# CompVis/retrieval-augmented-diffusion-models

Hardware: AMD Instinct MI355X
Metric: images/sec at 256x256, 50 DDIM steps, k=4 OpenImages retrieval (higher is better)
Workload: dtype bf16; 1 GPU; BASELINE config #3: RDM sampling, exact kNN (k=4) over a synthetic 20927907 x 512 fp16 CLIP DB -> 50-step DDIM (eta 0, CFG scale 2.0) over the shipped-config UNet (400.9M params, random weights) -> VQ-f4 decode to 256x256; batch_per_gpu=64, global_batch=64, sampler_steps=50, k=4, db_rows=20927907, parallelism=dp1 (batch-sharded, weights + DB replicated, all-gather of images only), deterministic_mode=False

## Files before the change

retrieval-augmented-diffusion-models_amd/csrc/conv_halo4.hip:

```cpp

#include <type_traits>

#include "kernels.h"

__device__ unsigned long long g_halo4_prof[4];

__global__ __launch_bounds__(256) void conv_w_fragpack_kernel(const bf16_t* __restrict__ W, bf16_t* __restrict__ dst, int N, int Cin) {
    const int KQ = Cin >> 4;
    const long long nvec = (long long)N * 9 * Cin / 8;
    for (long long v = (long long)blockIdx.x * 256 + threadIdx.x; v < nvec; v += (long long)gridDim.x * 256) {
        const int lane = (int)(v & 63);
        long long f = v >> 6;
        const int kq = (int)(f % KQ); f /= KQ;
        const int tap = (int)(f % 9); const int nb = (int)(f / 9);
        const int n = nb * 32 + (lane & 31), c = kq * 16 + (lane >> 5) * 8;
        *(uint4*)(dst + v * 8) = *(const uint4*)(W + ((long long)n * 9 + tap) * Cin + c);
    }
}
hipError_t launch_conv_w_fragpack(const bf16_t* W, bf16_t* dst, int N, int Cin, hipStream_t st) {
    const long long nvec = (long long)N * 9 * Cin / 8;
    long long g = (nvec + 255) / 256; if (g > 8192) g = 8192;
    conv_w_fragpack_kernel<<<dim3((unsigned)g), 256, 0, st>>>(W, dst, N, Cin);
    return hipGetLastError();
}
// ... 186 lines not shown
    }
    slice_setup();
    typedef __attribute__((ext_vector_type(4))) unsigned u32x4_t;
    union FragU { u32x4_t u; bf16x8 f; };
    auto start_values = [&](int tm0, int tn0, int row, float (&pb)[FM][FN]) {
#pragma unroll
        for (int i = 0; i < FM; i++) {
            const int mf = tm0 + wm * 128 + i * 32;
            const float* rv = p.rowvec ? p.rowvec + (long long)(mf / p.rows_per_sample) * p.rowvec_ld : nullptr;
#pragma unroll
            for (int j = 0; j < FN; j++) {
                const int ncol = tn0 + wn * WN + j * 32 + row;
                float bv = (S == 1 && p.bias) ? p.bias[ncol] : 0.f;
                if (S == 1 && rv) bv += rv[ncol];
                pb[i][j] = bv;
            }
        }
    };
    auto start_frag = [&](float bv, int half) -> bf16x8 {
        const uint32_t hi = cvt_pk_bf16(bv, 0.f) & 0xffffu;
        const uint32_t lo = cvt_pk_bf16(bv - __uint_as_float(hi << 16), 0.f) & 0xffffu;
        FragU t; t.u = (u32x4_t){half ? 0u : (hi | (lo << 16)), 0u, 0u, 0u};
        return t.f;
    };
    {
        float pb[FM][FN];
        start_values(em0, en0, frow, pb);
        FragU o; o.u = (u32x4_t){fhalf ? 0u : 0x3f803f80u, 0u, 0u, 0u};
        bf16x8 ones = o.f;
#pragma unroll
        for (int i = 0; i < FM; i++) {
            bf16x8 sf[FN];
#pragma unroll
            for (int j = 0; j < FN; j++) sf[j] = start_frag(pb[i][j], fhalf);
            if constexpr (FN == 3) asm volatile("s_nop 7" : "+v"(sf[0]), "+v"(sf[1]), "+v"(sf[2]), "+v"(ones));
            else asm volatile("s_nop 7" : "+v"(sf[0]), "+v"(sf[1]), "+v"(ones));
#pragma unroll
            for (int j = 0; j < FN; j++) H4_MFMA0(i * FN + j, sf[j], ones);
        }
    }

    unsigned long long tprof[2] = {0, 0};
    unsigned long long tp0 = 0, tp1 = 0;
    if (p.dbg & 16) tp0 = __builtin_readcyclecounter();
    bool slice_last_tap = false;
    int epi_stores = 0;
    const char* sbn = Wf; unsigned noff = 0; int q0 = 0;
    auto describe = [&]() {
        slice_last_tap = tap == 8;
        const int n_tap = slice_last_tap ? 0 : tap + 1;
        sbn = slice_last_tap ? sb_after : sb_run + tap_stride;
        sb_run = sbn;
        const int ndy = (n_tap * 11) >> 5, ndx = n_tap - ndy * 3;
        noff = (slice_last_tap ? hbase_nxt : hbase_cur) + (unsigned)(ndy * RSTR + ndx * 144);
        q0 = tap * 3;
    };
    auto step = [&](auto ptag) {
        constexpr int P = decltype(ptag)::value;
        auto mfma = [&](int ks, int m) {
            const int j = m / FM, i = m % FM;
            H4_MFMA(i * FN + j, fb[P][ks][j], fa[ks & 1][i]);
        };
        if (epi_stores == 0) asm volatile("s_waitcnt vmcnt(3) lgkmcnt(0)" ::: "memory");
        else if (epi_stores == FM * ((32 * (WN / 8)) / 64)) asm volatile("s_waitcnt vmcnt(%0) lgkmcnt(0)" :: "i"(3 + FM * ((32 * (WN / 8)) / 64)) : "memory");
        else asm volatile("s_waitcnt vmcnt(%0) lgkmcnt(0)" :: "i"(3 + 4 * FM * FN) : "memory");
        epi_stores = 0;
        H4_LDSW(hdst[P][0], hreg[P][0]);
#pragma unroll
        for (int m = 0; m < FM * FN; m++) {
            mfma(0, m);
            H4_GLOADB(fb[P ^ 1][m / FN][m % FN], voffj[m % FN], sbn, (m / FN) * 1024);
            if (m == 3) {
#pragma unroll
                for (int i = 0; i < FM; i++) H4_LDSR(fa[1][i], va[i], 32);
            }
        }
#pragma unroll
        for (int ks = 1; ks < 4; ks++) {
            asm volatile("s_waitcnt lgkmcnt(0)" ::: "memory");
            if (ks < 3) H4_LDSW(hdst[P][ks], hreg[P][ks]);
            const int q = q0 + ks - 1;
            const bool live = q < hnp;
            unsigned pe;
            asm volatile("ds_read_b32 %0, %1" : "=v"(pe) : "v"(tbl + (unsigned)((q < 20 ? q : 20) * 256)));
            mfma(ks, 0); mfma(ks, 1); mfma(ks, 2); mfma(ks, 3);
            if (ks < 3) {
#pragma unroll
                for (int i = 0; i < FM; i++) H4_LDSR(fa[(ks + 1) & 1][i], va[i], (ks + 1) * 32);
            } else {
                if (slice_last_tap) __builtin_amdgcn_s_barrier();
#pragma unroll
                for (int i = 0; i < FM; i++) { va[i] = vbase[i] + noff; H4_LDSR(fa[0][i], va[i], 0); }
            }
            asm volatile("s_waitcnt lgkmcnt(4)" : "+v"(pe) :: "memory");
            mfma(ks, 4);
            int hy = (int)((pe >> 20) & 63u), sp = (int)((pe >> 26) & 3u), xs = (int)((pe >> 13) & (STRIP ? 127u : 63u));
            if constexpr (STRIP) xs += ht_x0(ht) - 1;
            H4_PIN3(hy, sp, xs);
            mfma(ks, 5);
            int y = ht_y0(ht) + hy - 1;
            const bool xin = STRIP ? ((unsigned)xs < (unsigned)WI) : (((pe >> 19) & 1u) != 0);
            unsigned okm = (live & xin & ((unsigned)y < (unsigned)H)) ? 0xffffffffu : 0u;
            if constexpr (STRIP) xs >>= ups;
            H4_PIN2(y, okm);
            mfma(ks, 6);
            int t = __mul24(ht.b0 + sp, p.Hin) + (y >> ups);
            H4_PIN1(t);
            mfma(ks, 7);
            unsigned pix = (unsigned)__mul24(t, p.Win) + (unsigned)xs;
            unsigned long long ga = (unsigned long long)hs.src + (unsigned long long)pix * hs.ldb + (unsigned)(lc * 16);
            unsigned glo = (unsigned)ga, ghi = (unsigned)(ga >> 32);
            H4_PIN2(glo, ghi);
            if constexpr (FN >= 3) mfma(ks, 8);
            const unsigned long long zb = (unsigned long long)zl;
            glo = (glo & okm) | ((unsigned)zb & ~okm); ghi = (ghi & okm) | ((unsigned)(zb >> 32) & ~okm);
            H4_PIN2(glo, ghi);
            if constexpr (FN >= 3) mfma(ks, 9);
            unsigned hd = hbase_nxt + ((pe & 0x1fffu) << 4);
            hd = (live & (((pe >> 28) & 1u) != 0)) ? hd : dump;
            H4_PIN1(hd);
            const char* hg = (const char*)(((unsigned long long)ghi << 32) | glo);
            if constexpr (FN >= 3) mfma(ks, 10);
            H4_GLOADH(hreg[P][ks - 1], hg); hdst[P][ks - 1] = hd;
            if constexpr (FN >= 3) mfma(ks, 11);
        }
    };
    auto advance = [&]() -> bool {
        if (!slice_last_tap) { tap++; return false; }
        tap = 0; hb ^= 1; sl++;
        if (sl < s_end) { slice_setup(); return false; }

        if (!has_next) asm volatile("s_waitcnt vmcnt(0) lgkmcnt(0)" ::: "memory");
        asm volatile("s_nop 15\n\ts_nop 15" ::: "memory");

        if (p.dbg & 16) { tp1 = __builtin_readcyclecounter(); tprof[0] += tp1 - tp0; }
        char* const stg_base = smem + (hb ^ 1) * HBYTES;
        int lane_e = lane;
        asm volatile("" : "+v"(lane_e));
        const int erow = lane_e & 31, ehalf = lane_e >> 5;
        constexpr int CPR = WN / 8, NIT = (32 * CPR) / 64;
        static_assert((32 * CPR) % 64 == 0, "epilogue staging geometry");
        const bool swz = HBYTES < 4 * 32 * (WN * 4 + 16);
        const int SROW = swz ? WN * 4 : WN * 4 + 16;
        const unsigned stg0 = (unsigned)((hb ^ 1) * HBYTES + wave * 32 * SROW);
        const unsigned fw = swz ? (unsigned)((erow >> 1) & 7) : 0u;
        unsigned stgw[4];
#pragma unroll
        for (int g = 0; g < 4; g++) stgw[g] = stg0 + (unsigned)(erow * SROW) + ((((unsigned)(2 * g + ehalf)) ^ fw) << 4);
        const int eno = en0 + wn * WN;
        float pb[FM][FN];
        start_values(nem0, nen0, erow, pb);
        FragU o1; o1.u = (u32x4_t){ehalf ? 0u : 0x3f803f80u, 0u, 0u, 0u};
        bf16x8 ones = o1.f;
        auto stage_row = [&](int i) {
#pragma unroll
            for (int j = 0; j < FN; j++) {
                H4_LDSW_ACC(stgw[0], i * FN + j, 0, j * 128); H4_LDSW_ACC(stgw[1], i * FN + j, 1, j * 128);
                H4_LDSW_ACC(stgw[2], i * FN + j, 2, j * 128); H4_LDSW_ACC(stgw[3], i * FN + j, 3, j * 128);
            }
            bf16x8 sf[FN];
#pragma unroll
            for (int j = 0; j < FN; j++) sf[j] = start_frag(pb[i][j], ehalf);
            if constexpr (FN == 3) asm volatile("s_waitcnt lgkmcnt(0)\n\ts_nop 7" : "+v"(sf[0]), "+v"(sf[1]), "+v"(sf[2]), "+v"(ones) :: "memory");
            else asm volatile("s_waitcnt lgkmcnt(0)\n\ts_nop 7" : "+v"(sf[0]), "+v"(sf[1]), "+v"(ones) :: "memory");
#pragma unroll
            for (int j = 0; j < FN; j++) H4_MFMA0(i * FN + j, sf[j], ones);
        };
        if (S > 1) {
            constexpr int CPR4 = WN / 4, NIT4 = (32 * CPR4) / 64;
            unsigned voffs[NIT4], lrd4[NIT4];
#pragma unroll
            for (int it = 0; it < NIT4; it++) {
                const int idx = it * 64 + lane_e, row = idx / CPR4, c4 = idx - row * CPR4;
                voffs[it] = (unsigned)(row * p.N + c4 * 4) * 4u;
                const unsigned fr = swz ? (unsigned)((row >> 1) & 7) : 0u;
                lrd4[it] = stg0 + (unsigned)(row * SROW) + ((((unsigned)c4 & ~7u) | (((unsigned)c4 ^ fr) & 7u)) << 4);
            }
            const char* const wbase = (const char*)(p.ws + (long long)part * p.M * p.N + (long long)(em0 + wm * 128) * p.N + eno);
            const unsigned long long rowstep = (unsigned long long)(32 * p.N) * 4ull;
#pragma unroll
            for (int i = 0; i < FM; i++) {
                stage_row(i);
                const char* const op = (const char*)h4_uni64((unsigned long long)(wbase + i * rowstep));
#pragma unroll
                for (int it = 0; it < NIT4; it++) {
                    const float4 a0 = *(const float4*)(smem + lrd4[it]);
                    const h4_u32x4 d0 = {__float_as_uint(a0.x), __float_as_uint(a0.y), __float_as_uint(a0.z), __float_as_uint(a0.w)};
                    H4_GSTORES(voffs[it], d0, op);
                }
            }
        } else {
            unsigned voffs[NIT], lrd[NIT];
#pragma unroll
            for (int it = 0; it < NIT; it++) {
                const int idx = it * 64 + lane_e, row = idx / CPR, ch = idx - row * CPR;
                voffs[it] = (unsigned)(row * p.ldo + ch * 8) * 2u;
                const unsigned fr = swz ? (unsigned)((row >> 1) & 7) : 0u, c4 = (unsigned)(2 * ch);
                lrd[it] = stg0 + (unsigned)(row * SROW) + (((c4 & ~7u) | ((c4 ^ fr) & 7u)) << 4);
            }
            const unsigned lx = swz ? 16u : 0u, la = swz ? 0u : 16u;
            auto frag_row0 = [&](int i) -> long long {
                if constexpr (STRIP) {
                    const int tp = wm * 128 + i * 32;
                    return ((long long)(ht_tile.b0 * H + ht_y0(ht_tile) + (tp >> 6)) * WI + ht_x0(ht_tile) + (tp & 63));
                } else return (long long)(em0 + wm * 128 + i * 32);
            };
            const char* const obase = (const char*)(ob + eno);
            const char* const rbase = (const char*)(rb + eno);
            const unsigned long long rowbytes = (unsigned long long)p.ldo * 2ull;
            h4_u32x4 rr4[2][NIT];
            auto res_request = [&](int i, h4_u32x4 (&dst)[NIT]) {
                const char* const rp = (const char*)h4_uni64((unsigned long long)(rbase + (unsigned long long)frag_row0(i) * rowbytes));
#pragma unroll
                for (int it = 0; it < NIT; it++) H4_GLOADB(dst[it], voffs[it], rp, 0);
            };
            auto res_wait = [&](h4_u32x4 (&r)[NIT], auto ntag) {
                constexpr int N = decltype(ntag)::value;
#pragma unroll
                for (int it = 0; it < NIT; it++) asm volatile("" : "+v"(r[it]));
                asm volatile("s_waitcnt vmcnt(%0)" :: "i"(N) : "memory");
#pragma unroll
                for (int it = 0; it < NIT; it++) asm volatile("" : "+v"(r[it]));
            };
            auto store_row = [&](int i) {
                const char* const op = (const char*)h4_uni64((unsigned long long)(obase + (unsigned long long)frag_row0(i) * rowbytes));
#pragma unroll
                for (int it = 0; it < NIT; it++) {
                    float4 a0 = *(const float4*)(smem + lrd[it]), a1 = *(const float4*)(smem + ((lrd[it] ^ lx) + la));
                    if (rb) {
                        const h4_u32x4 r4 = rr4[i & 1][it];
                        a0.x += __uint_as_float(r4.x << 16); a0.y += __uint_as_float(r4.x & 0xffff0000u);
                        a0.z += __uint_as_float(r4.y << 16); a0.w += __uint_as_float(r4.y & 0xffff0000u);
                        a1.x += __uint_as_float(r4.z << 16); a1.y += __uint_as_float(r4.z & 0xffff0000u);
                        a1.z += __uint_as_float(r4.w << 16); a1.w += __uint_as_float(r4.w & 0xffff0000u);
                    }
                    const h4_u32x4 dv = {cvt_pk_bf16(a0.x, a0.y), cvt_pk_bf16(a0.z, a0.w), cvt_pk_bf16(a1.x, a1.y), cvt_pk_bf16(a1.z, a1.w)};
                    H4_GSTORES(voffs[it], dv, op);
                }
            };
            if (rb) {
                res_request(0, rr4[0]); res_request(1, rr4[1]);
                stage_row(0); res_wait(rr4[0], std::integral_constant<int, NIT>{}); store_row(0);
                res_request(2, rr4[0]);
                stage_row(1); res_wait(rr4[1], std::integral_constant<int, 2 * NIT>{}); store_row(1);
                res_request(3, rr4[1]);
                stage_row(2); res_wait(rr4[0], std::integral_constant<int, 2 * NIT>{}); store_row(2);
                stage_row(3); res_wait(rr4[1], std::integral_constant<int, NIT>{}); store_row(3);
            } else {
                stage_row(0); store_row(0);
                stage_row(1); store_row(1);
                stage_row(2); store_row(2);
                stage_row(3); store_row(3);
            }
        }
        epi_stores = (S > 1) ? 2 * FM * ((32 * (WN / 8)) / 64) : FM * ((32 * (WN / 8)) / 64);
        if (p.dbg & 16) tprof[1] += __builtin_readcyclecounter() - tp1;
        if (!has_next) return true;
        __builtin_amdgcn_s_barrier();
        tile = next;
        tile_setup();
        sl = s_begin;
        slice_setup();
        if (p.dbg & 16) tp0 = __builtin_readcyclecounter();
        return false;
    };
    while (true) {
        describe(); step(std::integral_constant<int, 0>{}); if (advance()) break;
        describe(); step(std::integral_constant<int, 1>{}); if (advance()) break;
    }
    if ((p.dbg & 16) && tid == 0) {
        atomicAdd(&g_halo4_prof[0], tprof[0]); atomicAdd(&g_halo4_prof[1], tprof[1]); atomicAdd(&g_halo4_prof[3], 1ull);
    }
}

template <int FN, bool STRIP = false>
static hipError_t launch_halo4_cfg(const IgemmParams& p, hipStream_t st) {
    constexpr int smem = 2 * H4_HALO_MAX + 4096 + 4 * 21 * 256;
    constexpr int BN = FN * 64;
    static int ncu_dev[RDM_MAX_DEVICES] = {0};
    const int dev = rdm_cur_device();
    if (!ncu_dev[dev]) {
        hipError_t e = hipFuncSetAttribute((const void*)conv3x3_halo4_kernel<FN, STRIP>, hipFuncAttributeMaxDynamicSharedMemorySize, smem);
        if (e != hipSuccess) return e;
        hipDeviceGetAttribute(&ncu_dev[dev], hipDeviceAttributeMultiprocessorCount, dev);
    }
    const int ncu = ncu_dev[dev];
    const long long ntiles = (long long)(p.M / 256) * (p.N / BN) * (p.ksplit > 1 ? p.ksplit : 1);
    long long g = (ncu + 7) & ~7;
    if (g > ntiles) g = ntiles;
    conv3x3_halo4_kernel<FN, STRIP><<<dim3((unsigned)g), 256, smem, st>>>(p);
    return hipGetLastError();
}

hipError_t launch_conv_halo4(const IgemmParams& p, bool strip, hipStream_t st) {
    if (strip) return launch_halo4_cfg<2, true>(p, st);
    if (p.N % 192 == 0) return launch_halo4_cfg<3>(p, st);
    return launch_halo4_cfg<2>(p, st);
}
```

retrieval-augmented-diffusion-models_amd/csrc/h4_asm.h:

```cpp
#pragma once
#include "common.h"

#define H4_ACC0 64
#define H4_ACC_CLOBBERS "a64","a65","a66","a67","a68","a69","a70","a71","a72","a73","a74","a75","a76","a77","a78","a79","a80","a81","a82","a83","a84","a85","a86","a87","a88","a89","a90","a91","a92","a93","a94","a95","a96","a97","a98","a99","a100","a101","a102","a103","a104","a105","a106","a107","a108","a109","a110","a111","a112","a113","a114","a115","a116","a117","a118","a119","a120","a121","a122","a123","a124","a125","a126","a127","a128","a129","a130","a131","a132","a133","a134","a135","a136","a137","a138","a139","a140","a141","a142","a143","a144","a145","a146","a147","a148","a149","a150","a151","a152","a153","a154","a155","a156","a157","a158","a159","a160","a161","a162","a163","a164","a165","a166","a167","a168","a169","a170","a171","a172","a173","a174","a175","a176","a177","a178","a179","a180","a181","a182","a183","a184","a185","a186","a187","a188","a189","a190","a191","a192","a193","a194","a195","a196","a197","a198","a199","a200","a201","a202","a203","a204","a205","a206","a207","a208","a209","a210","a211","a212","a213","a214","a215","a216","a217","a218","a219","a220","a221","a222","a223","a224","a225","a226","a227","a228","a229","a230","a231","a232","a233","a234","a235","a236","a237","a238","a239","a240","a241","a242","a243","a244","a245","a246","a247","a248","a249","a250","a251","a252","a253","a254","a255"
#define H4_MFMA(IDX, a, b)  asm volatile("v_mfma_f32_32x32x16_bf16 a[%c2:%c3], %0, %1, a[%c2:%c3]" :: "v"(a), "v"(b), "i"(H4_ACC0 + (IDX) * 16), "i"(H4_ACC0 + (IDX) * 16 + 15))
#define H4_MFMA0(IDX, a, b) asm volatile("v_mfma_f32_32x32x16_bf16 a[%c2:%c3], %0, %1, 0" :: "v"(a), "v"(b), "i"(H4_ACC0 + (IDX) * 16), "i"(H4_ACC0 + (IDX) * 16 + 15))
#define H4_ACCZERO(IDX, R) asm volatile("v_accvgpr_write_b32 a%c0, 0" :: "i"(H4_ACC0 + (IDX) * 16 + (R)))
#define H4_ACCREAD(dst, IDX, R) asm volatile("v_accvgpr_read_b32 %0, a%c1" : "=v"(dst) : "i"(H4_ACC0 + (IDX) * 16 + (R)))
#define H4_LDSR(dst, addr, off)  asm volatile("ds_read_b128 %0, %1 offset:%2" : "=v"(dst) : "v"(addr), "i"(off))
#define H4_LDSW(addr, src)  asm volatile("ds_write_b128 %0, %1" :: "v"(addr), "v"(src) : "memory")
#define H4_GLOADB(dst, voff, sbase, imm) asm volatile("global_load_dwordx4 %0, %1, %2 offset:%3" : "=v"(dst) : "v"(voff), "s"(sbase), "i"(imm) : "memory")
#define H4_GLOADH(dst, vaddr) asm volatile("global_load_dwordx4 %0, %1, off" : "=v"(dst) : "v"(vaddr) : "memory")
typedef __attribute__((ext_vector_type(4))) unsigned h4_u32x4;
#define H4_GSTORE(vaddr, data) asm volatile("global_store_dwordx4 %0, %1, off\n\ts_nop 1" :: "v"(vaddr), "v"(data) : "memory")
#define H4_PIN1(a) asm volatile("" : "+v"(a))
#define H4_PIN2(a, b) asm volatile("" : "+v"(a), "+v"(b))
#define H4_PIN3(a, b, c) asm volatile("" : "+v"(a), "+v"(b), "+v"(c))
#define H4_GSTOREO(vaddr, data, off) asm volatile("global_store_dwordx4 %0, %1, off offset:%2\n\ts_nop 1" :: "v"(vaddr), "v"(data), "i"(off) : "memory")
#define H4_GSTORES(voff, data, sbase) asm volatile("global_store_dwordx4 %0, %1, %2\n\ts_nop 1" :: "v"(voff), "v"(data), "s"(sbase) : "memory")
#define H4_GSTORES_NT(voff, data, sbase) asm volatile("global_store_dwordx4 %0, %1, %2 nt\n\ts_nop 1" :: "v"(voff), "v"(data), "s"(sbase) : "memory")
#define H4_GSTORESO(voff, data, sbase, off) asm volatile("global_store_dwordx4 %0, %1, %2 offset:%3\n\ts_nop 1" :: "v"(voff), "v"(data), "s"(sbase), "i"(off) : "memory")
__device__ __forceinline__ unsigned long long h4_uni64(unsigned long long v) {
    const unsigned lo = __builtin_amdgcn_readfirstlane((unsigned)v), hi = __builtin_amdgcn_readfirstlane((unsigned)(v >> 32));
    return ((unsigned long long)hi << 32) | lo;
}
#define H4_GLOADB_A(AIDX, voff, sbase) asm volatile("global_load_dwordx4 a[%c0:%c1], %2, %3" :: "i"(AIDX), "i"((AIDX) + 3), "v"(voff), "s"(sbase) : "memory")
#define H4_AREAD(dst, AIDX) asm volatile("v_accvgpr_read_b32 %0, a%c1" : "=v"(dst) : "i"(AIDX))
#define H4_LDSW_ACC(addr, IDX, G, off) asm volatile("ds_write_b128 %0, a[%c1:%c2] offset:%3" :: "v"(addr), "i"(H4_ACC0 + (IDX) * 16 + (G) * 4), "i"(H4_ACC0 + (IDX) * 16 + (G) * 4 + 3), "i"(off) : "memory")
#define H4_ACCWRITE(IDX, R, src) asm volatile("v_accvgpr_write_b32 a%c0, %1" :: "i"(H4_ACC0 + (IDX) * 16 + (R)), "v"(src))
#define H4_LDSWO(addr, src, off)  asm volatile("ds_write_b128 %0, %1 offset:%2" :: "v"(addr), "v"(src), "i"(off) : "memory")
#define H4_PERMSWAP(a, b) asm volatile("v_permlane32_swap_b32 %0, %1" : "+v"(a), "+v"(b))
```

retrieval-augmented-diffusion-models_amd/csrc/lin4.hip:

```cpp

#include <type_traits>

#include "kernels.h"
#include "h4_asm.h"

__host__ __device__ inline int l4_geglu_row(int n) {
    const int nb = n >> 5, fr = n & 31;
    return 64 * (nb >> 1) + 16 * (nb & 1) + (fr < 16 ? fr : 32 + (fr - 16));
}
__global__ __launch_bounds__(256) void lin_w_fragpack_kernel(const bf16_t* __restrict__ W, bf16_t* __restrict__ dst, int N, int K, int ldw, int geglu,
                                                             const float* __restrict__ gamma) {
    const int KQ = K >> 4;
    const long long nvec = (long long)N * K / 8;
    for (long long v = (long long)blockIdx.x * 256 + threadIdx.x; v < nvec; v += (long long)gridDim.x * 256) {
        const int lane = (int)(v & 63);
        const long long f = v >> 6;
        const int kq = (int)(f % KQ), nb = (int)(f / KQ);
        int n = nb * 32 + (lane & 31);
        const int c = kq * 16 + (lane >> 5) * 8;
        if (geglu) n = l4_geglu_row(n);
        uint4 w = *(const uint4*)(W + (long long)n * ldw + c);
        if (gamma) {
            uint32_t* u = (uint32_t*)&w;
#pragma unroll
// ... 153 lines not shown
                const int g = i >= p.N ? 1 : 0, n = i - g * p.N;
                const float bv = ((long long)g * p.rows_per_sample < p.M) ? p.rowvec[(long long)g * p.rowvec_ld + (GEGLU ? l4_geglu_row(n) : n)] : 0.f;
                const uint32_t hi = cvt_pk_bf16(bv, 0.f) & 0xffffu;
                const uint32_t lo = cvt_pk_bf16(bv - __uint_as_float(hi << 16), 0.f) & 0xffffu;
                *(uint32_t*)(smem + L4_RV + i * 4) = hi | (lo << 16);
            }
        }
    }
    __syncthreads();
    typedef __attribute__((ext_vector_type(4))) unsigned u32x4_t;
    union FragU { u32x4_t u; bf16x8 f; };
    auto bias_frags = [&](int bn, int bm, int row, int half, bf16x8 (&bf)[FN], bf16x8& ones) __attribute__((always_inline)) {
        const int rvoff = L4_RV + ((bm * BM >= rv_split) ? p.N * 4 : 0);
#pragma unroll
        for (int j = 0; j < FN; j++) {
            uint32_t w = 0u, w2 = 0u;
            if constexpr (!LN) {
                w = *(const uint32_t*)(smem + L4_BIAS + (bn * BN + wn * WN + j * 32 + row) * 4);
                if (has_rv) w2 = *(const uint32_t*)(smem + rvoff + (bn * BN + wn * WN + j * 32 + row) * 4);
            }
            FragU t; t.u = (u32x4_t){half ? 0u : w, half ? 0u : w2, 0u, 0u};
            bf[j] = t.f;
        }
        FragU o; o.u = (u32x4_t){half ? 0u : 0x3f803f80u, half ? 0u : 0x3f803f80u, 0u, 0u};
        ones = o.f;
    };
    auto acc_init = [&](int bn, int bm) __attribute__((always_inline)) {
        bf16x8 bf[FN], ones;
        bias_frags(bn, bm, frow, fhalf, bf, ones);
        asm volatile("s_nop 7" : "+v"(bf[0]), "+v"(bf[1]), "+v"(bf[2]), "+v"(ones));
#pragma unroll
        for (int i = 0; i < FM; i++)
#pragma unroll
            for (int j = 0; j < FN; j++) H4_MFMA0(i * FN + j, bf[j], ones);
    };

    {
        ASrc s0 = a_src(ca); cur_adv(ca);
#pragma unroll
        for (int q = 0; q < NPC; q++) H4_GLOADB(hreg[0][q], s0.voff, s0.base + (unsigned)q * s0.pstride, 0);
        asm volatile("s_waitcnt vmcnt(0)" ::: "memory");
#pragma unroll
        for (int q = 0; q < NPC; q++) { H4_LDSWO(ldsw0, hreg[0][q], q * 4608); stat_half(q, hreg[0][q], 0); stat_half(q, hreg[0][q], 1); }
        ASrc s1 = a_src(ca); cur_adv(ca);
#pragma unroll
        for (int q = 0; q < NPC; q++) H4_GLOADB(hreg[0][q], s1.voff, s1.base + (unsigned)q * s1.pstride, 0);
        const char* sb = w_base(cb); cur_adv(cb);
#pragma unroll
        for (int ks = 0; ks < 4; ks++)
#pragma unroll
            for (int j = 0; j < FN; j++) { H4_GLOADB(fb[0][ks][j], voffj[j], sb, ks * 1024); fb[1][ks][j] = fb[0][ks][j]; }
        ASrc s2 = a_src(ca); cur_adv(ca);
#pragma unroll
        for (int q = 0; q < NPC; q++) H4_GLOADB(hreg[1][q], s2.voff, s2.base + (unsigned)q * s2.pstride, 0);
        asm volatile("s_waitcnt lgkmcnt(0)" ::: "memory");
        __builtin_amdgcn_s_barrier();
#pragma unroll
        for (int i = 0; i < FM; i++) { H4_LDSR(fa[0][i], vbase[i], 0); fa[1][i] = fa[0][i]; }
    }
    acc_init(cc.bn, cc.bm);

    int epi_stores = 0;
    const char* sbn = Wf; ASrc an{zero, 0u, lane16};
    auto describe = [&]() __attribute__((always_inline)) {
        sbn = (const char*)l4_uni64((unsigned long long)((cb.tile < t_end) ? w_base(cb) : Wf));
        cur_adv(cb);
        an = a_src(ca);
        cur_adv(ca);
    };
    auto step = [&](auto ptag) __attribute__((always_inline)) {
        constexpr int P = decltype(ptag)::value;
        constexpr int RB = P * L4_ABUF;
        auto mfma = [&](int ks, int m) {
            const int j = m / FM, i = m % FM;
            H4_MFMA(i * FN + j, fb[P][ks][j], fa[ks & 1][i]);
        };
        if (epi_stores == 0) asm volatile("s_waitcnt vmcnt(%0) lgkmcnt(0)" :: "i"(NPC) : "memory");
        else asm volatile("s_waitcnt vmcnt(%0) lgkmcnt(0)" :: "i"(NPC + (GEGLU ? FM * FN : 2 * FM * FN)) : "memory");
        epi_stores = 0;
#pragma unroll
        for (int m = 0; m < FM * FN; m++) {
            mfma(0, m);
            H4_GLOADB(fb[P ^ 1][m / FN][m % FN], voffj[m % FN], sbn, (m / FN) * 1024);
            if (m == 3) {
#pragma unroll
                for (int i = 0; i < FM; i++) H4_LDSR(fa[1][i], vbase[i], RB + 32);
            }
        }
#pragma unroll
        for (int ks = 1; ks < 4; ks++) {
            const int q0 = NPC == 8 ? (ks - 1) * 3 : (ks == 1 ? 0 : ks), nq = NPC == 8 ? (ks < 3 ? 3 : 2) : (ks == 1 ? 2 : 1);
            asm volatile("s_waitcnt lgkmcnt(0)" ::: "memory");
#pragma unroll
            for (int q = q0; q < q0 + nq; q++) {
                if (P == 0) H4_LDSWO(ldsw1, hreg[P][q], q * 4608); else H4_LDSWO(ldsw0, hreg[P][q], q * 4608);
            }
            auto stat_at = [&](int m) __attribute__((always_inline)) { if (m < 2 * nq) stat_half(q0 + (m >> 1), hreg[P][q0 + (m >> 1)], m & 1); };
            mfma(ks, 0); stat_at(0); mfma(ks, 1); stat_at(1); mfma(ks, 2); stat_at(2); mfma(ks, 3); stat_at(3);
            if (ks < 3) {
#pragma unroll
                for (int i = 0; i < FM; i++) H4_LDSR(fa[(ks + 1) & 1][i], vbase[i], RB + (ks + 1) * 32);
            } else {
                asm volatile("s_waitcnt lgkmcnt(0)" ::: "memory");
                __builtin_amdgcn_s_barrier();
#pragma unroll
                for (int i = 0; i < FM; i++) H4_LDSR(fa[0][i], vbase[i], (P ^ 1) * L4_ABUF);
            }
            mfma(ks, 4); stat_at(4); mfma(ks, 5); stat_at(5);
#pragma unroll
            for (int q = q0; q < q0 + nq; q++) {
                H4_GLOADB(hreg[P][q], an.voff, an.base + (unsigned)q * an.pstride, 0);
                mfma(ks, 6 + 2 * (q - q0)); mfma(ks, 7 + 2 * (q - q0));
            }
            if (nq <= 2) { mfma(ks, 10); mfma(ks, 11); }
            if (nq == 1) { mfma(ks, 8); mfma(ks, 9); }
        }
    };

    auto advance = [&]() __attribute__((always_inline)) -> bool {
        const int sl_done = cc.sl;
        if (sl_done + 1 < nslice) {
            cc.sl++;
            if constexpr (LN) {
                if (cc.sl == nslice - 1) {
#pragma unroll
                    for (int q = 0; q < NPC; q++) {
                        float sv = lsum[q], tv = lsq[q];
                        sv += __builtin_bit_cast(float, __builtin_amdgcn_update_dpp(0, __builtin_bit_cast(int, sv), 0xB1, 0xf, 0xf, true));
                        tv += __builtin_bit_cast(float, __builtin_amdgcn_update_dpp(0, __builtin_bit_cast(int, tv), 0xB1, 0xf, 0xf, true));
                        sv += __builtin_bit_cast(float, __builtin_amdgcn_update_dpp(0, __builtin_bit_cast(int, sv), 0x4E, 0xf, 0xf, true));
                        tv += __builtin_bit_cast(float, __builtin_amdgcn_update_dpp(0, __builtin_bit_cast(int, tv), 0x4E, 0xf, 0xf, true));
                        sv += __builtin_bit_cast(float, __builtin_amdgcn_update_dpp(0, __builtin_bit_cast(int, sv), 0x141, 0xf, 0xf, true));
                        tv += __builtin_bit_cast(float, __builtin_amdgcn_update_dpp(0, __builtin_bit_cast(int, tv), 0x141, 0xf, 0xf, true));
                        const float mean = sv * p.ln_inv_c;
                        const float var = fmaxf(tv * p.ln_inv_c - mean * mean, 0.f);
                        const float rstd = __builtin_amdgcn_rsqf(var + p.ln_eps);
                        if (lc == 0) *(float2*)(smem + L4_STAT + ((q * 4 + wave) * 8 + lp) * 8) = make_float2(mean, rstd);
                        lsum[q] = 0.f; lsq[q] = 0.f;
                    }
                }
            }
            return false;
        }
        const int em0 = cc.bm * BM, en0 = cc.bn * BN;
        Cur nx = cc; cur_adv(nx);
        const bool has_next = nx.tile < t_end;
        if (!has_next) asm volatile("s_waitcnt vmcnt(0) lgkmcnt(0)" ::: "memory");
        asm volatile("s_nop 15\n\ts_nop 15" ::: "memory");

        int lane_e = lane;
        asm volatile("" : "+v"(lane_e));
        const int erow = lane_e & 31, ehalf = lane_e >> 5;
        const unsigned stgw = (unsigned)(L4_STG + wave * (32 * 400) + erow * 400 + ehalf * 16);
        const char* const stgr = smem + L4_STG + wave * (32 * 400);
        bf16x8 nbf[FN], nones;
        if constexpr (LN) {
            FragU z; z.u = (u32x4_t){0u, 0u, 0u, 0u};
            nones = z.f;
        } else {
            bias_frags(has_next ? nx.bn : cc.bn, has_next ? nx.bm : cc.bm, erow, ehalf, nbf, nones);
        }
        if constexpr (LN) { asm volatile("" : "+v"(nones)); nbf[0] = nones; nbf[1] = nones; nbf[2] = nones; }
        else asm volatile("" : "+v"(nbf[0]), "+v"(nbf[1]), "+v"(nbf[2]), "+v"(nones));
        auto stage_row = [&](int i) __attribute__((always_inline)) {
#pragma unroll
            for (int j = 0; j < FN; j++) {
                H4_LDSW_ACC(stgw, i * FN + j, 0, (j * 8 + 0) * 16); H4_LDSW_ACC(stgw, i * FN + j, 1, (j * 8 + 2) * 16);
                H4_LDSW_ACC(stgw, i * FN + j, 2, (j * 8 + 4) * 16); H4_LDSW_ACC(stgw, i * FN + j, 3, (j * 8 + 6) * 16);
            }
            asm volatile("s_waitcnt lgkmcnt(0)" ::: "memory");
#pragma unroll
            for (int j = 0; j < FN; j++) H4_MFMA0(i * FN + j, nbf[j], nones);
        };
        if constexpr (GEGLU) {
            const int eno_o = (en0 >> 1) + wn * (WN / 2);
            unsigned voffs[3], lrd[3], sbo[3], srow[3];
#pragma unroll
            for (int it = 0; it < 3; it++) {
                const int idx = it * 64 + lane_e, row = idx / 6, c6 = idx - row * 6;
                voffs[it] = (unsigned)(row * ldo + c6 * 8) * 2u;
                lrd[it] = (unsigned)(row * 400 + ((c6 >> 1) * 32 + (c6 & 1) * 8) * 4);
                sbo[it] = (unsigned)(L4_BIAS + (en0 + wn * WN + (c6 >> 1) * 32 + (c6 & 1) * 8) * 8);
                srow[it] = (unsigned)(L4_STAT + (wm * 128 + row) * 8);
            }
            const char* const obase = (const char*)(ob + (long long)(em0 + wm * 128) * ldo + eno_o);
            const unsigned long long rowstep = (unsigned long long)(32 * ldo) * 2ull;
            auto store_row = [&](int i) __attribute__((always_inline)) {
                const char* const op = (const char*)l4_uni64((unsigned long long)(obase + i * rowstep));
#pragma unroll
                for (int it = 0; it < 3; it++) {
                    float4 x0 = *(const float4*)(stgr + lrd[it]), x1 = *(const float4*)(stgr + lrd[it] + 16);
                    float4 g0 = *(const float4*)(stgr + lrd[it] + 64), g1 = *(const float4*)(stgr + lrd[it] + 80);
                    if constexpr (LN) {
                        const float2 st = *(const float2*)(smem + srow[it] + i * 256);
                        const float r = st.y, m2 = -st.x * st.y;
                        const float4* const qx = (const float4*)(smem + sbo[it]); const float4* const qg = (const float4*)(smem + sbo[it] + 128);
                        const float4 a = qx[0], b = qx[1], c = qx[2], d = qx[3];
                        x0.x = fmaf(r, x0.x, fmaf(m2, a.x, a.y)); x0.y = fmaf(r, x0.y, fmaf(m2, a.z, a.w));
                        x0.z = fmaf(r, x0.z, fmaf(m2, b.x, b.y)); x0.w = fmaf(r, x0.w, fmaf(m2, b.z, b.w));
                        x1.x = fmaf(r, x1.x, fmaf(m2, c.x, c.y)); x1.y = fmaf(r, x1.y, fmaf(m2, c.z, c.w));
                        x1.z = fmaf(r, x1.z, fmaf(m2, d.x, d.y)); x1.w = fmaf(r, x1.w, fmaf(m2, d.z, d.w));
                        const float4 e = qg[0], f = qg[1], g = qg[2], h = qg[3];
                        g0.x = fmaf(r, g0.x, fmaf(m2, e.x, e.y)); g0.y = fmaf(r, g0.y, fmaf(m2, e.z, e.w));
                        g0.z = fmaf(r, g0.z, fmaf(m2, f.x, f.y)); g0.w = fmaf(r, g0.w, fmaf(m2, f.z, f.w));
                        g1.x = fmaf(r, g1.x, fmaf(m2, g.x, g.y)); g1.y = fmaf(r, g1.y, fmaf(m2, g.z, g.w));
                        g1.z = fmaf(r, g1.z, fmaf(m2, h.x, h.y)); g1.w = fmaf(r, g1.w, fmaf(m2, h.z, h.w));
                    }
                    const f32x2_t r0 = (f32x2_t){x0.x, x0.y} * gelu_erf_f2((f32x2_t){g0.x, g0.y});
                    const f32x2_t r1 = (f32x2_t){x0.z, x0.w} * gelu_erf_f2((f32x2_t){g0.z, g0.w});
                    const f32x2_t r2 = (f32x2_t){x1.x, x1.y} * gelu_erf_f2((f32x2_t){g1.x, g1.y});
                    const f32x2_t r3 = (f32x2_t){x1.z, x1.w} * gelu_erf_f2((f32x2_t){g1.z, g1.w});
                    const h4_u32x4 dv = {cvt_pk_bf16(r0.x, r0.y), cvt_pk_bf16(r1.x, r1.y), cvt_pk_bf16(r2.x, r2.y), cvt_pk_bf16(r3.x, r3.y)};
                    H4_GSTORES_NT(voffs[it], dv, op);
                }
            };
            stage_row(0); store_row(0);
            stage_row(1); store_row(1);
            stage_row(2); store_row(2);
            stage_row(3); store_row(3);
        } else {
            const int eno = en0 + wn * WN;
            unsigned voffs[6], lrd[6], sbo[3], srow[3];
#pragma unroll
            for (int it = 0; it < 6; it++) {
                const int idx = it * 64 + lane_e, row = idx / 12, ch = idx - row * 12;
                voffs[it] = (unsigned)(row * ldo + ch * 8) * 2u;
                lrd[it] = (unsigned)(row * 400 + ch * 32);
                if (it < 3) { sbo[it] = (unsigned)(L4_BIAS + (en0 + wn * WN + ch * 8) * 8); srow[it] = (unsigned)(L4_STAT + (wm * 128 + row) * 8); }
            }
            const char* const obase = (const char*)(ob + (long long)(em0 + wm * 128) * ldo + eno);
            const int er0 = (p.res_wrap_rows > 0 && em0 >= p.res_wrap_rows) ? em0 - p.res_wrap_rows : em0;
            const char* const rbase = (const char*)(rb + (long long)(er0 + wm * 128) * ldo + eno);
            const unsigned long long rowstep = (unsigned long long)(32 * ldo) * 2ull;
            h4_u32x4 rr4[2][6];
            auto res_request = [&](int i, h4_u32x4 (&dst)[6]) __attribute__((always_inline)) {
                const char* const rp = (const char*)l4_uni64((unsigned long long)(rbase + i * rowstep));
#pragma unroll
                for (int it = 0; it < 6; it++) H4_GLOADB(dst[it], voffs[it], rp, 0);
            };
            auto store_row = [&](int i) __attribute__((always_inline)) {
                const char* const op = (const char*)l4_uni64((unsigned long long)(obase + i * rowstep));
#pragma unroll
                for (int it = 0; it < 6; it++) {
                    float4 a0 = *(const float4*)(stgr + lrd[it]), a1 = *(const float4*)(stgr + lrd[it] + 16);
                    if constexpr (LN) {
                        const float2 st = *(const float2*)(smem + srow[it % 3] + i * 256 + (it / 3) * 128);
                        const float r = st.y, m2 = -st.x * st.y;
                        const float4* const qs = (const float4*)(smem + sbo[it % 3]);
                        const float4 a = qs[0], b = qs[1], c = qs[2], d = qs[3];
                        a0.x = fmaf(r, a0.x, fmaf(m2, a.x, a.y)); a0.y = fmaf(r, a0.y, fmaf(m2, a.z, a.w));
                        a0.z = fmaf(r, a0.z, fmaf(m2, b.x, b.y)); a0.w = fmaf(r, a0.w, fmaf(m2, b.z, b.w));
                        a1.x = fmaf(r, a1.x, fmaf(m2, c.x, c.y)); a1.y = fmaf(r, a1.y, fmaf(m2, c.z, c.w));
                        a1.z = fmaf(r, a1.z, fmaf(m2, d.x, d.y)); a1.w = fmaf(r, a1.w, fmaf(m2, d.z, d.w));
                    }
                    if (!LN && rb) {
                        const h4_u32x4 r4 = rr4[i & 1][it];
                        a0.x += __uint_as_float(r4.x << 16); a0.y += __uint_as_float(r4.x & 0xffff0000u);
                        a0.z += __uint_as_float(r4.y << 16); a0.w += __uint_as_float(r4.y & 0xffff0000u);
                        a1.x += __uint_as_float(r4.z << 16); a1.y += __uint_as_float(r4.z & 0xffff0000u);
                        a1.z += __uint_as_float(r4.w << 16); a1.w += __uint_as_float(r4.w & 0xffff0000u);
                    }
                    const h4_u32x4 dv = {cvt_pk_bf16(a0.x, a0.y), cvt_pk_bf16(a0.z, a0.w), cvt_pk_bf16(a1.x, a1.y), cvt_pk_bf16(a1.z, a1.w)};
                    H4_GSTORES(voffs[it], dv, op);
                }
            };
            constexpr int NST = 6;
            if (!LN && rb) {
                res_request(0, rr4[0]); res_request(1, rr4[1]);
                stage_row(0);
                asm volatile("s_waitcnt vmcnt(6)" : "+v"(rr4[0][0]), "+v"(rr4[0][1]), "+v"(rr4[0][2]), "+v"(rr4[0][3]), "+v"(rr4[0][4]), "+v"(rr4[0][5]) :: "memory");
                store_row(0);
                res_request(2, rr4[0]);
                stage_row(1);
                asm volatile("s_waitcnt vmcnt(%6)" : "+v"(rr4[1][0]), "+v"(rr4[1][1]), "+v"(rr4[1][2]), "+v"(rr4[1][3]), "+v"(rr4[1][4]), "+v"(rr4[1][5]) : "i"(6 + NST) : "memory");
                store_row(1);
                res_request(3, rr4[1]);
                stage_row(2);
                asm volatile("s_waitcnt vmcnt(%6)" : "+v"(rr4[0][0]), "+v"(rr4[0][1]), "+v"(rr4[0][2]), "+v"(rr4[0][3]), "+v"(rr4[0][4]), "+v"(rr4[0][5]) : "i"(6 + NST) : "memory");
                store_row(2);
                stage_row(3);
                asm volatile("s_waitcnt vmcnt(%6)" : "+v"(rr4[1][0]), "+v"(rr4[1][1]), "+v"(rr4[1][2]), "+v"(rr4[1][3]), "+v"(rr4[1][4]), "+v"(rr4[1][5]) : "i"(NST) : "memory");
                store_row(3);
            } else {
                stage_row(0); store_row(0);
                stage_row(1); store_row(1);
                stage_row(2); store_row(2);
                stage_row(3); store_row(3);
            }
        }
        epi_stores = GEGLU ? FM * FN : 2 * FM * FN;
        if (!has_next) return true;
        cc = nx;
        return false;
    };
    while (true) {
        describe(); step(std::integral_constant<int, 0>{}); if (advance()) break;
        describe(); step(std::integral_constant<int, 1>{}); if (advance()) break;
    }
}

static int lin4_wm(const IgemmParams& p) {
    if (p.N % 384 == 0 && p.M % 128 == 0) return 1;
    if (p.N % 192 == 0 && p.M % 256 == 0) return 2;
    return 0;
}
static int lin4_smem_bytes(const IgemmParams& p, int wm) {
    return 2 * (128 * wm * 144) + 4 * 32 * 400 + (p.ln_sb ? p.N * 8 + 128 * wm * 8 : p.N * 4 + (p.rowvec ? 2 * p.N * 4 : 0));
}
bool lin4_supported(const IgemmParams& p, int batch) {
    if (!p.Wfrag || batch != 1) return false;
    const int wm = lin4_wm(p);
    if (!wm || p.K % 64 || p.C0 % 64 || p.C1 % 64 || p.K != p.C0 + p.C1) return false;
    if (p.alpha != 1.0f || p.res_f32 || p.out_f32 || !p.out_bf16) return false;
    if (p.rowvec && (p.ln_sb || p.rows_per_sample <= 0 || p.rows_per_sample % (128 * wm) != 0 || 2LL * p.rows_per_sample < p.M || p.rowvec_ld < p.N)) return false;
    const bool geglu = p.act == ACT_GEGLU;
    if (p.act != ACT_NONE && !geglu) return false;
    if (geglu && p.res_bf16) return false;
    const int No = geglu ? p.N / 2 : p.N;
    if (p.N > 8192 || p.ldo % 8 || p.ldo < No || (p.ldw > 0 && p.ldw != p.K)) return false;
    if (p.C1 > 0 && p.lda > 0) return false;
    if (p.res_wrap_rows > 0 && (!p.res_bf16 || p.res_wrap_rows % (128 * wm) != 0 || 2LL * p.res_wrap_rows < p.M)) return false;
    if (p.a1_wrap_rows > 0 && (p.C1 == 0 || p.a1_wrap_rows % (128 * wm) != 0 || 2LL * p.a1_wrap_rows < p.M)) return false;
    if (p.ln_sb && (p.C1 > 0 || p.K < 128 || p.res_bf16 || p.bias || lin4_smem_bytes(p, wm) > 160 * 1024 || !(p.ln_inv_c > 0.f))) return false;
    constexpr int L4_MIN_TILES = 128;
    if (!p.l4_any_tiles && (long long)(p.M / (128 * wm)) * (p.N / (wm == 1 ? 384 : 192)) < L4_MIN_TILES) return false;
    return true;
}

template <bool GEGLU, int WM, bool LN>
static hipError_t launch_lin4_cfg(const IgemmParams& p, hipStream_t st) {
    const int smem = lin4_smem_bytes(p, WM);
    static int ncu_dev[RDM_MAX_DEVICES] = {0};
    const int dev = rdm_cur_device();
    if (!ncu_dev[dev]) {
        hipError_t e = hipFuncSetAttribute((const void*)lin4_kernel<GEGLU, WM, LN>, hipFuncAttributeMaxDynamicSharedMemorySize, 160 * 1024);
        if (e != hipSuccess) return e;
        hipDeviceGetAttribute(&ncu_dev[dev], hipDeviceAttributeMultiprocessorCount, dev);
    }
    const long long ntiles = (long long)(p.M / (128 * WM)) * (p.N / (WM == 1 ? 384 : 192));
    long long g = (ncu_dev[dev] + 7) & ~7;
    if (g > ntiles) g = ntiles;
    lin4_kernel<GEGLU, WM, LN><<<dim3((unsigned)g), 256, smem, st>>>(p);
    return hipGetLastError();
}
hipError_t launch_lin4(const IgemmParams& p, hipStream_t st) {
    const int wm = lin4_wm(p);
    if (p.ln_sb) {
        if (p.act == ACT_GEGLU) return wm == 1 ? launch_lin4_cfg<true, 1, true>(p, st) : launch_lin4_cfg<true, 2, true>(p, st);
        return wm == 1 ? launch_lin4_cfg<false, 1, true>(p, st) : launch_lin4_cfg<false, 2, true>(p, st);
    }
    if (p.act == ACT_GEGLU) return wm == 1 ? launch_lin4_cfg<true, 1, false>(p, st) : launch_lin4_cfg<true, 2, false>(p, st);
    return wm == 1 ? launch_lin4_cfg<false, 1, false>(p, st) : launch_lin4_cfg<false, 2, false>(p, st);
}
```

Baseline: 42.45 images/s.

## Software-pipeline epilogue LDS staging reads and next-row accumulator writes

Restructures the epilogues of the halo4 conv and lin4 GEMM kernels. LDS readbacks of the staged accumulators now go through explicit asm reads in a rolling window, and the next row's accumulator-to-LDS writes are issued before the current row's global stores finish. Partial lgkmcnt waits replace the full lgkmcnt(0) drains, so LDS latency can overlap global stores and MFMA-based requantization. This adds fragile hand-counted waitcnt bookkeeping. Any miscount or write-after-read hazard on the staging buffer would give wrong results.

```diff
diff --git a/retrieval-augmented-diffusion-models_amd/csrc/conv_halo4.hip b/retrieval-augmented-diffusion-models_amd/csrc/conv_halo4.hip
--- a/retrieval-augmented-diffusion-models_amd/csrc/conv_halo4.hip
+++ b/retrieval-augmented-diffusion-models_amd/csrc/conv_halo4.hip
@@ -362,17 +362,21 @@
         start_values(nem0, nen0, erow, pb);
         FragU o1; o1.u = (u32x4_t){ehalf ? 0u : 0x3f803f80u, 0u, 0u, 0u};
         bf16x8 ones = o1.f;
-        auto stage_row = [&](int i) {
+        constexpr int NSW = 4 * FN;
+        auto stage_writes = [&](int i) __attribute__((always_inline)) {
 #pragma unroll
             for (int j = 0; j < FN; j++) {
                 H4_LDSW_ACC(stgw[0], i * FN + j, 0, j * 128); H4_LDSW_ACC(stgw[1], i * FN + j, 1, j * 128);
                 H4_LDSW_ACC(stgw[2], i * FN + j, 2, j * 128); H4_LDSW_ACC(stgw[3], i * FN + j, 3, j * 128);
             }
+        };
+        auto stage_finish = [&](int i, auto ytag) __attribute__((always_inline)) {
+            constexpr int YOUNGER = decltype(ytag)::value;
             bf16x8 sf[FN];
 #pragma unroll
             for (int j = 0; j < FN; j++) sf[j] = start_frag(pb[i][j], ehalf);
-            if constexpr (FN == 3) asm volatile("s_waitcnt lgkmcnt(0)\n\ts_nop 7" : "+v"(sf[0]), "+v"(sf[1]), "+v"(sf[2]), "+v"(ones) :: "memory");
-            else asm volatile("s_waitcnt lgkmcnt(0)\n\ts_nop 7" : "+v"(sf[0]), "+v"(sf[1]), "+v"(ones) :: "memory");
+            if constexpr (FN == 3) asm volatile("s_waitcnt lgkmcnt(%4)\n\ts_nop 7" : "+v"(sf[0]), "+v"(sf[1]), "+v"(sf[2]), "+v"(ones) : "i"(YOUNGER) : "memory");
+            else asm volatile("s_waitcnt lgkmcnt(%3)\n\ts_nop 7" : "+v"(sf[0]), "+v"(sf[1]), "+v"(ones) : "i"(YOUNGER) : "memory");
 #pragma unroll
             for (int j = 0; j < FN; j++) H4_MFMA0(i * FN + j, sf[j], ones);
         };
@@ -388,15 +392,24 @@
             }
             const char* const wbase = (const char*)(p.ws + (long long)part * p.M * p.N + (long long)(em0 + wm * 128) * p.N + eno);
             const unsigned long long rowstep = (unsigned long long)(32 * p.N) * 4ull;
+            constexpr int RW4 = 4;
+            h4_f32x4 sp[RW4];
+            stage_writes(0);
 #pragma unroll
             for (int i = 0; i < FM; i++) {
-                stage_row(i);
+#pragma unroll
+                for (int it = 0; it < RW4; it++) H4_LDSR(sp[it], lrd4[it], 0);
+                stage_finish(i, std::integral_constant<int, RW4>{});
                 const char* const op = (const char*)h4_uni64((unsigned long long)(wbase + i * rowstep));
 #pragma unroll
                 for (int it = 0; it < NIT4; it++) {
-                    const float4 a0 = *(const float4*)(smem + lrd4[it]);
+                    const int ahead = ((NIT4 - 1 - it) < (RW4 - 1) ? (NIT4 - 1 - it) : (RW4 - 1)) + ((i < FM - 1 && it > NIT4 - 3) ? NSW : 0);
+                    H4_LDSWAIT1(sp[it % RW4], ahead);
+                    const h4_f32x4 a0 = sp[it % RW4];
                     const h4_u32x4 d0 = {__float_as_uint(a0.x), __float_as_uint(a0.y), __float_as_uint(a0.z), __float_as_uint(a0.w)};
                     H4_GSTORES(voffs[it], d0, op);
+                    if (it + RW4 < NIT4) H4_LDSR(sp[(it + RW4) % RW4], lrd4[it + RW4], 0);
+                    if (i < FM - 1 && it == NIT4 - 3) stage_writes(i + 1);
                 }
             }
         } else {
@@ -432,11 +445,26 @@
 #pragma unroll
                 for (int it = 0; it < NIT; it++) asm volatile("" : "+v"(r[it]));
             };
-            auto store_row = [&](int i) {
+            constexpr int RW = FN == 3 ? 2 : 3;
+            static_assert(NIT > RW && 2 + NSW <= 15, "read-out window / lgkmcnt range");
+            h4_f32x4 sa0[RW], sa1[RW];
+            auto rd_issue = [&](int it) __attribute__((always_inline)) {
+                const unsigned l1 = (lrd[it] ^ lx) + la;
+                H4_LDSR(sa0[it % RW], lrd[it], 0); H4_LDSR(sa1[it % RW], l1, 0);
+            };
+            auto stage_row = [&](int i) __attribute__((always_inline)) {
+                if (i == 0) stage_writes(0);
+#pragma unroll
+                for (int it = 0; it < RW; it++) rd_issue(it);
+                stage_finish(i, std::integral_constant<int, 2 * RW>{});
+            };
+            auto store_row = [&](int i) __attribute__((always_inline)) {
                 const char* const op = (const char*)h4_uni64((unsigned long long)(obase + (unsigned long long)frag_row0(i) * rowbytes));
 #pragma unroll
                 for (int it = 0; it < NIT; it++) {
-                    float4 a0 = *(const float4*)(smem + lrd[it]), a1 = *(const float4*)(smem + ((lrd[it] ^ lx) + la));
+                    const int ahead = 2 * ((NIT - 1 - it) < (RW - 1) ? (NIT - 1 - it) : (RW - 1)) + ((i < FM - 1 && it > NIT - 3) ? NSW : 0);
+                    H4_LDSWAIT2(sa0[it % RW], sa1[it % RW], ahead);
+                    h4_f32x4 a0 = sa0[it % RW], a1 = sa1[it % RW];
                     if (rb) {
                         const h4_u32x4 r4 = rr4[i & 1][it];
                         a0.x += __uint_as_float(r4.x << 16); a0.y += __uint_as_float(r4.x & 0xffff0000u);
@@ -446,6 +474,8 @@
                     }
                     const h4_u32x4 dv = {cvt_pk_bf16(a0.x, a0.y), cvt_pk_bf16(a0.z, a0.w), cvt_pk_bf16(a1.x, a1.y), cvt_pk_bf16(a1.z, a1.w)};
                     H4_GSTORES(voffs[it], dv, op);
+                    if (it + RW < NIT) rd_issue(it + RW);
+                    if (i < FM - 1 && it == NIT - 3) stage_writes(i + 1);
                 }
             };
             if (rb) {
diff --git a/retrieval-augmented-diffusion-models_amd/csrc/h4_asm.h b/retrieval-augmented-diffusion-models_amd/csrc/h4_asm.h
--- a/retrieval-augmented-diffusion-models_amd/csrc/h4_asm.h
+++ b/retrieval-augmented-diffusion-models_amd/csrc/h4_asm.h
@@ -30,3 +30,7 @@
 #define H4_ACCWRITE(IDX, R, src) asm volatile("v_accvgpr_write_b32 a%c0, %1" :: "i"(H4_ACC0 + (IDX) * 16 + (R)), "v"(src))
 #define H4_LDSWO(addr, src, off)  asm volatile("ds_write_b128 %0, %1 offset:%2" :: "v"(addr), "v"(src), "i"(off) : "memory")
 #define H4_PERMSWAP(a, b) asm volatile("v_permlane32_swap_b32 %0, %1" : "+v"(a), "+v"(b))
+typedef __attribute__((ext_vector_type(4))) float h4_f32x4;
+#define H4_LDSWAIT1(a, N) asm volatile("s_waitcnt lgkmcnt(%1)" : "+v"(a) : "i"(N))
+#define H4_LDSWAIT2(a, b, N) asm volatile("s_waitcnt lgkmcnt(%2)" : "+v"(a), "+v"(b) : "i"(N))
+#define H4_LDSWAIT4(a, b, c, d, N) asm volatile("s_waitcnt lgkmcnt(%4)" : "+v"(a), "+v"(b), "+v"(c), "+v"(d) : "i"(N))
diff --git a/retrieval-augmented-diffusion-models_amd/csrc/lin4.hip b/retrieval-augmented-diffusion-models_amd/csrc/lin4.hip
--- a/retrieval-augmented-diffusion-models_amd/csrc/lin4.hip
+++ b/retrieval-augmented-diffusion-models_amd/csrc/lin4.hip
@@ -329,7 +329,8 @@
         asm volatile("" : "+v"(lane_e));
         const int erow = lane_e & 31, ehalf = lane_e >> 5;
         const unsigned stgw = (unsigned)(L4_STG + wave * (32 * 400) + erow * 400 + ehalf * 16);
-        const char* const stgr = smem + L4_STG + wave * (32 * 400);
+        const unsigned stgr = (unsigned)(L4_STG + wave * (32 * 400));
+        constexpr int NSW = 4 * FN;
         bf16x8 nbf[FN], nones;
         if constexpr (LN) {
             FragU z; z.u = (u32x4_t){0u, 0u, 0u, 0u};
@@ -339,13 +340,15 @@
         }
         if constexpr (LN) { asm volatile("" : "+v"(nones)); nbf[0] = nones; nbf[1] = nones; nbf[2] = nones; }
         else asm volatile("" : "+v"(nbf[0]), "+v"(nbf[1]), "+v"(nbf[2]), "+v"(nones));
-        auto stage_row = [&](int i) __attribute__((always_inline)) {
+        auto stage_writes = [&](int i) __attribute__((always_inline)) {
 #pragma unroll
             for (int j = 0; j < FN; j++) {
                 H4_LDSW_ACC(stgw, i * FN + j, 0, (j * 8 + 0) * 16); H4_LDSW_ACC(stgw, i * FN + j, 1, (j * 8 + 2) * 16);
                 H4_LDSW_ACC(stgw, i * FN + j, 2, (j * 8 + 4) * 16); H4_LDSW_ACC(stgw, i * FN + j, 3, (j * 8 + 6) * 16);
             }
-            asm volatile("s_waitcnt lgkmcnt(0)" ::: "memory");
+        };
+        auto stage_finish = [&](int i, int younger) __attribute__((always_inline)) {
+            asm volatile("s_waitcnt lgkmcnt(%0)" :: "i"(younger) : "memory");
 #pragma unroll
             for (int j = 0; j < FN; j++) H4_MFMA0(i * FN + j, nbf[j], nones);
         };
@@ -356,18 +359,29 @@
             for (int it = 0; it < 3; it++) {
                 const int idx = it * 64 + lane_e, row = idx / 6, c6 = idx - row * 6;
                 voffs[it] = (unsigned)(row * ldo + c6 * 8) * 2u;
-                lrd[it] = (unsigned)(row * 400 + ((c6 >> 1) * 32 + (c6 & 1) * 8) * 4);
+                lrd[it] = stgr + (unsigned)(row * 400 + ((c6 >> 1) * 32 + (c6 & 1) * 8) * 4);
                 sbo[it] = (unsigned)(L4_BIAS + (en0 + wn * WN + (c6 >> 1) * 32 + (c6 & 1) * 8) * 8);
                 srow[it] = (unsigned)(L4_STAT + (wm * 128 + row) * 8);
             }
             const char* const obase = (const char*)(ob + (long long)(em0 + wm * 128) * ldo + eno_o);
             const unsigned long long rowstep = (unsigned long long)(32 * ldo) * 2ull;
+            constexpr int NST = 3, RW = 2;
+            h4_f32x4 sx0[RW], sx1[RW], sg0[RW], sg1[RW];
+            auto rd_issue = [&](int it) __attribute__((always_inline)) {
+                H4_LDSR(sx0[it % RW], lrd[it], 0); H4_LDSR(sx1[it % RW], lrd[it], 16);
+                H4_LDSR(sg0[it % RW], lrd[it], 64); H4_LDSR(sg1[it % RW], lrd[it], 80);
+            };
+            auto rd_first = [&]() __attribute__((always_inline)) {
+#pragma unroll
+                for (int it = 0; it < RW; it++) rd_issue(it);
+            };
             auto store_row = [&](int i) __attribute__((always_inline)) {
                 const char* const op = (const char*)l4_uni64((unsigned long long)(obase + i * rowstep));
 #pragma unroll
-                for (int it = 0; it < 3; it++) {
-                    float4 x0 = *(const float4*)(stgr + lrd[it]), x1 = *(const float4*)(stgr + lrd[it] + 16);
-                    float4 g0 = *(const float4*)(stgr + lrd[it] + 64), g1 = *(const float4*)(stgr + lrd[it] + 80);
+                for (int it = 0; it < NST; it++) {
+                    const int ahead = 4 * ((NST - 1 - it) < (RW - 1) ? (NST - 1 - it) : (RW - 1)) + ((i < FM - 1 && it > NST - 2) ? NSW : 0);
+                    H4_LDSWAIT4(sx0[it % RW], sx1[it % RW], sg0[it % RW], sg1[it % RW], ahead);
+                    h4_f32x4 x0 = sx0[it % RW], x1 = sx1[it % RW], g0 = sg0[it % RW], g1 = sg1[it % RW];
                     if constexpr (LN) {
                         const float2 st = *(const float2*)(smem + srow[it] + i * 256);
                         const float r = st.y, m2 = -st.x * st.y;
@@ -389,12 +403,14 @@
                     const f32x2_t r3 = (f32x2_t){x1.z, x1.w} * gelu_erf_f2((f32x2_t){g1.z, g1.w});
                     const h4_u32x4 dv = {cvt_pk_bf16(r0.x, r0.y), cvt_pk_bf16(r1.x, r1.y), cvt_pk_bf16(r2.x, r2.y), cvt_pk_bf16(r3.x, r3.y)};
                     H4_GSTORES_NT(voffs[it], dv, op);
+                    if (it + RW < NST) rd_issue(it + RW);
+                    if (i < FM - 1 && it == NST - 2) stage_writes(i + 1);
                 }
             };
-            stage_row(0); store_row(0);
-            stage_row(1); store_row(1);
-            stage_row(2); store_row(2);
-            stage_row(3); store_row(3);
+            stage_writes(0); rd_first(); stage_finish(0, 4 * RW); store_row(0);
+            rd_first(); stage_finish(1, 4 * RW); store_row(1);
+            rd_first(); stage_finish(2, 4 * RW); store_row(2);
+            rd_first(); stage_finish(3, 4 * RW); store_row(3);
         } else {
             const int eno = en0 + wn * WN;
             unsigned voffs[6], lrd[6], sbo[3], srow[3];
@@ -402,7 +418,7 @@
             for (int it = 0; it < 6; it++) {
                 const int idx = it * 64 + lane_e, row = idx / 12, ch = idx - row * 12;
                 voffs[it] = (unsigned)(row * ldo + ch * 8) * 2u;
-                lrd[it] = (unsigned)(row * 400 + ch * 32);
+                lrd[it] = stgr + (unsigned)(row * 400 + ch * 32);
                 if (it < 3) { sbo[it] = (unsigned)(L4_BIAS + (en0 + wn * WN + ch * 8) * 8); srow[it] = (unsigned)(L4_STAT + (wm * 128 + row) * 8); }
             }
             const char* const obase = (const char*)(ob + (long long)(em0 + wm * 128) * ldo + eno);
@@ -415,11 +431,20 @@
 #pragma unroll
                 for (int it = 0; it < 6; it++) H4_GLOADB(dst[it], voffs[it], rp, 0);
             };
+            constexpr int NST = 6, RW = 3;
+            h4_f32x4 sa0[RW], sa1[RW];
+            auto rd_issue = [&](int it) __attribute__((always_inline)) { H4_LDSR(sa0[it % RW], lrd[it], 0); H4_LDSR(sa1[it % RW], lrd[it], 16); };
+            auto rd_first = [&]() __attribute__((always_inline)) {
+#pragma unroll
+                for (int it = 0; it < RW; it++) rd_issue(it);
+            };
             auto store_row = [&](int i) __attribute__((always_inline)) {
                 const char* const op = (const char*)l4_uni64((unsigned long long)(obase + i * rowstep));
 #pragma unroll
-                for (int it = 0; it < 6; it++) {
-                    float4 a0 = *(const float4*)(stgr + lrd[it]), a1 = *(const float4*)(stgr + lrd[it] + 16);
+                for (int it = 0; it < NST; it++) {
+                    const int ahead = 2 * ((NST - 1 - it) < (RW - 1) ? (NST - 1 - it) : (RW - 1)) + ((i < FM - 1 && it > NST - 3) ? NSW : 0);
+                    H4_LDSWAIT2(sa0[it % RW], sa1[it % RW], ahead);
+                    h4_f32x4 a0 = sa0[it % RW], a1 = sa1[it % RW];
                     if constexpr (LN) {
                         const float2 st = *(const float2*)(smem + srow[it % 3] + i * 256 + (it / 3) * 128);
                         const float r = st.y, m2 = -st.x * st.y;
@@ -439,9 +464,15 @@
                     }
                     const h4_u32x4 dv = {cvt_pk_bf16(a0.x, a0.y), cvt_pk_bf16(a0.z, a0.w), cvt_pk_bf16(a1.x, a1.y), cvt_pk_bf16(a1.z, a1.w)};
                     H4_GSTORES(voffs[it], dv, op);
+                    if (it + RW < NST) rd_issue(it + RW);
+                    if (i < FM - 1 && it == NST - 3) stage_writes(i + 1);
                 }
             };
-            constexpr int NST = 6;
+            auto stage_row = [&](int i) __attribute__((always_inline)) {
+                if (i == 0) stage_writes(0);
+                rd_first();
+                stage_finish(i, 2 * RW);
+            };
             if (!LN && rb) {
                 res_request(0, rr4[0]); res_request(1, rr4[1]);
                 stage_row(0);
```

Result: no change. 42.59 images/s (median of 6 runs) (+0.3%).
